# althonos/pyskani

Measured on AMD Instinct MI355X. Metric: genome-pairs/sec (sketch+ANI), higher is better.
Workload: dtype u64; 1 GPU; all-vs-all 10000 x 10000 synthetic ~5 Mb genomes on one GPU (100 families x 100; single-contig genomes, substitutions only), c=125 marker_c=1000 k=15; device-resident ASCII; hits=999867, genomes=10000, parallelism=references sharded over 1 GPU(s)

## Files before the change

pyskani_amd/csrc/slice_join.hip:

```cpp
#include "slice_join.h"
#include "chain_dev.h"

void gsl_make_tab(const BatchQ* bq, size_t n_entries, const uint32_t* q_seeds, std::vector<uint2>& tab, std::vector<uint2>& ebase, uint64_t* n_records, uint64_t* n_slices) {
    tab.clear(); ebase.resize(n_entries);
    uint64_t rec = 0, nsl_all = 0; uint32_t max_sl = 0;
    for (size_t e = 0; e < n_entries; e++) {
        const uint32_t nsl = (q_seeds[e] + GSL_SEEDS - 1) / GSL_SEEDS;
        ebase[e] = make_uint2((uint32_t)rec, (uint32_t)nsl_all);
        rec += (uint64_t)nsl * (bq[e].rank_hi - bq[e].rank_lo);
        nsl_all += nsl;
        max_sl = std::max(max_sl, nsl);
    }
    *n_records = rec; *n_slices = nsl_all;
    (void)max_sl;
    for (size_t e = 0; e < n_entries; e++) for (uint32_t sl = 0; sl < (q_seeds[e] + GSL_SEEDS - 1) / GSL_SEEDS; sl++) tab.push_back(make_uint2((uint32_t)e, sl));
}

#ifndef GSL_LINE_N
#define GSL_LINE_N 4
#endif
constexpr uint32_t GSL_LW = GSL_LINE_N, GSL_LM = GSL_LW - 1u, GSL_LS = GSL_LW == 8 ? 3u : GSL_LW == 4 ? 2u : 1u;
static_assert(GSL_LW == 8 || GSL_LW == 4 || GSL_LW == 2, "a staged line holds eight, four or two anchors");
static size_t gsl_walk_lds(const GslArgs& A, bool emit) {
    const size_t nw = (A.n_refs + 63) / 64;
    (void)nw;
    return (emit ? (8 * GSL_LW + 8 + 8) * (size_t)A.p_cap + 8 * 64 : 0) + 64 + 4 * (size_t)A.p_cap + (emit ? 0 : 4 * (size_t)GSL_WORDS * (A.p_cap + 1));
}

__device__ __forceinline__ uint32_t gsl_ref_word(unsigned long long v) { return (uint32_t)(v >> 53) & 7u; }
__device__ __forceinline__ uint32_t gsl_ref_bit(unsigned long long v) { return (uint32_t)(v >> 48) & 31u; }
__device__ __forceinline__ uint32_t gsl_tag(unsigned long long v) { return (uint32_t)(v >> 56); }
template <bool EMIT, bool TAGGED>
__global__ __launch_bounds__(64) void gsl_walk_kernel(GslArgs A) {
    extern __shared__ uint4 s_gsl[];
    const int lane = threadIdx.x;
    const uint2 te = A.tab[blockIdx.x];
    if (te.x == 0xFFFFFFFFu) return;
    if (EMIT && (A.err[5] || *(const unsigned long long*)(A.err + 16) > A.cap)) return;
    const BatchQ B = A.bq[te.x];
    const SketchDesc Q = A.qd[B.q];
    const uint32_t sb = te.y * GSL_SEEDS;
    if (sb >= Q.n) return;
    const uint32_t se = Q.n - sb > GSL_SEEDS ? sb + GSL_SEEDS : Q.n;
    const uint32_t P = B.rank_hi - B.rank_lo, pc = A.p_cap;
    const uint2 eb = A.ebase[te.x];
    const uint32_t rec0 = eb.x + te.y * P;
    uint2* s_line = (uint2*)s_gsl;
    unsigned long long* s_lim = (unsigned long long*)(s_line + (EMIT ? GSL_LW * pc : 0u));
    uint2* s_cs = (uint2*)(s_lim + (EMIT ? pc : 0u));
    uint2* s_fl = s_cs + (EMIT ? pc : 0u);
    uint2* s_bp = s_fl + (EMIT ? 64u : 0u);
    uint32_t* s_cur = (uint32_t*)(s_bp + 8u);
    uint32_t* s_rows = s_cur;
    uint32_t* s_bm = s_cur + pc;
    {
        if (EMIT) for (uint32_t j = lane; j < P; j += 64) { const uint4 v = A.rec[rec0 + j]; s_cs[j] = make_uint2(v.x, v.x); s_rows[j] = v.y; s_lim[j] = ((unsigned long long)v.w << 32) | v.z; }
        else {
            for (uint32_t j = lane; j < P; j += 64) s_cur[j] = 0;
            for (uint32_t x = lane; x < GSL_WORDS * (pc + 1u); x += 64) s_bm[x] = 0;
        }
    }
    uint32_t unw = 0;
    if (EMIT && lane < (int)GSL_WORDS) unw = A.un[(size_t)(eb.y + te.y) * GSL_WORDS + lane];
    lds_wave_sync();
    constexpr uint32_t GSL_AHEAD = 4;
    unsigned long long visited = 0;
    const uint32_t n_blk = A.blk_cnt[te.x];
    const uint32_t* __restrict__ brow = A.blk_tab + (size_t)te.x * A.blk_cap * GSL_BT_WORDS;
#pragma unroll 1
    for (uint32_t bi = 0; bi < n_blk; bi++, brow += GSL_BT_WORDS) {
    {
    const uint32_t blk = brow[8];
    const unsigned long long x_base = ((unsigned long long)brow[11] << 32) | brow[10];
    const uint32_t* __restrict__ x_key = A.g_key + x_base; const unsigned long long* __restrict__ x_val = A.g_val + x_base;
    {
        lds_wave_sync();
        if (lane < 8) {
            uint32_t run = brow[9];
#pragma unroll
            for (int u = 0; u < 7; u++) { const uint32_t w = brow[u]; if (u < lane) run += (uint32_t)__popc(w); }
            s_bp[lane] = make_uint2(brow[lane], run);
        }
        lds_wave_sync();
    }
    const uint32_t* __restrict__ bkt = A.g_bucket + (size_t)blk * A.g_nb1;
    uint32_t km1 = sb + (uint32_t)lane < se ? Q.kmer[sb + lane] : 0u, km2 = sb + 64u + (uint32_t)lane < se ? Q.kmer[sb + 64u + lane] : 0u;
    uint32_t lo1 = 0, hi1 = 0;
    if (sb + (uint32_t)lane < se) { const uint32_t b = km1 >> A.g_shift; lo1 = bkt[b]; hi1 = bkt[b + 1]; }
    for (uint32_t c0 = sb; c0 < se; c0 += 64) {
        const uint32_t i = c0 + (uint32_t)lane;
        const uint32_t km = km1, lo = lo1, hi = hi1;
        km1 = km2; lo1 = 0; hi1 = 0;
        if (i + 64u < se) { const uint32_t b = km1 >> A.g_shift; lo1 = bkt[b]; hi1 = bkt[b + 1]; }
        km2 = i + 128u < se ? Q.kmer[i + 128u] : 0u;
        uint32_t qp = 0, qm = 0;
        if (EMIT && i < se) { qp = Q.pos[i]; qm = Q.meta[i]; }
        const uint32_t nst = (hi - lo + 63u) >> 6;
        if (!EMIT) visited += hi - lo;
        uint32_t pre = nst;
#pragma unroll
        for (int o = 1; o < 64; o <<= 1) { const uint32_t y = __shfl_up(pre, o); if (lane >= o) pre += y; }
        const uint32_t T = (uint32_t)__builtin_amdgcn_readlane((int)pre, 63);
        pre -= nst;
        uint32_t ns[GSL_AHEAD], nx[GSL_AHEAD], nh[GSL_AHEAD], nk[GSL_AHEAD]; unsigned long long nv[GSL_AHEAD];
#define GSL_FETCH(t, u) do { \
            ns[u] = 0; nx[u] = 0; nh[u] = 0; nk[u] = 0xFFFFFFFFu; nv[u] = 0ull; \
            if ((t) < T) { \
                const unsigned long long own = __ballot(nst != 0 && pre <= (t)); \
                ns[u] = 63u - (uint32_t)__clzll((long long)own); \
                nx[u] = (uint32_t)__builtin_amdgcn_readlane((int)lo, (int)ns[u]) + 64u * ((t) - (uint32_t)__builtin_amdgcn_readlane((int)pre, (int)ns[u])); \
                nh[u] = (uint32_t)__builtin_amdgcn_readlane((int)hi, (int)ns[u]); \
                if (nx[u] + (uint32_t)lane < nh[u]) { if (!TAGGED) nk[u] = x_key[nx[u] + lane]; nv[u] = x_val[nx[u] + lane]; } \
            } } while (0)
#pragma unroll
        for (uint32_t u = 0; u < GSL_AHEAD; u++) GSL_FETCH(u, u);
        for (uint32_t t0 = 0; t0 < T; t0 += GSL_AHEAD) {
            uint32_t cs[GSL_AHEAD], cx[GSL_AHEAD], ch[GSL_AHEAD], ck[GSL_AHEAD]; unsigned long long cv[GSL_AHEAD];
#pragma unroll
            for (uint32_t u = 0; u < GSL_AHEAD; u++) { cs[u] = ns[u]; cx[u] = nx[u]; ch[u] = nh[u]; ck[u] = nk[u]; cv[u] = nv[u]; }
#pragma unroll
            for (uint32_t u = 0; u < GSL_AHEAD; u++) GSL_FETCH(t0 + GSL_AHEAD + u, u);
            uint32_t slots[GSL_AHEAD]; uint2 bps[GSL_AHEAD];
#pragma unroll
            for (uint32_t u = 0; u < GSL_AHEAD; u++) bps[u] = s_bp[gsl_ref_word(cv[u])];
#pragma unroll
            for (uint32_t u = 0; u < GSL_AHEAD; u++) {
                const uint32_t skm = (uint32_t)__builtin_amdgcn_readlane((int)km, (int)cs[u]);
                const uint32_t b = gsl_ref_bit(cv[u]), rk = bps[u].y + (uint32_t)__popc(bps[u].x & ~(~0u << b)) - B.rank_lo;
                const bool hit = TAGGED ? gsl_tag(cv[u]) == (skm & 0xFFu) : ck[u] == skm;
                const bool ok = cx[u] + (uint32_t)lane < ch[u] && hit && ((bps[u].x >> b) & 1u) && rk < P;
                slots[u] = ok ? rk : 0xFFFFFFFFu;
            }
#pragma unroll
            for (uint32_t u = 0; u < GSL_AHEAD; u++) {
                if (t0 + u >= T) break;
                const uint32_t s = cs[u]; const unsigned long long v = cv[u];
                const uint32_t slot = slots[u];
                const bool valid = slot != 0xFFFFFFFFu;
                if (!__any(valid)) continue;
                const uint32_t jl = c0 - sb + s;
                if (!EMIT) {
                    if (valid) { atomicAdd(&s_cur[slot], 1u); atomicOr(&s_bm[(jl >> 5) * (pc + 1u) + slot], 1u << (jl & 31u)); }
                    continue;
                }
                const uint32_t sqp = (uint32_t)__builtin_amdgcn_readlane((int)qp, (int)s), sqm = (uint32_t)__builtin_amdgcn_readlane((int)qm, (int)s);
                const uint32_t rmeta = (uint32_t)((((v >> 33) & ((1ull << GSI_CONTIG_BITS) - 1ull)) << 1) | (v & 1ull));
                const uint32_t prev = (uint32_t)__builtin_amdgcn_update_dpp(-1, (int)slot, 0x138 , 0xf, 0xf, false);
                const bool same = valid && prev == slot;
                const bool dup = __ballot(same) != 0;
                const uint2 cs = s_cs[valid ? slot : 0u];
                const unsigned long long lim = s_lim[valid ? slot : 0u];
                const uint32_t base = cs.x;
                bool opens = false;
                if (((uint32_t)__builtin_amdgcn_readlane((int)unw, (int)(jl >> 5)) >> (jl & 31u)) & 1u) {
                    const unsigned long long key1 = (((unsigned long long)(sqm >> 1) << 32) | sqp) + 1ull;
                    opens = valid && key1 > lim;
                    if (opens && !same) {
                        const uint32_t row = s_rows[slot], idxc = base < A.cap ? base : A.cap;
                        if (row < Q.rows) {
                            const size_t ri = (size_t)B.row_off + (size_t)slot * Q.rows + row;
                            uint2* r = A.chunks + ri;
                            r->x = idxc;
                            if (row > 0) r[-1].y = idxc;
                            A.row_q0[ri] = make_uint2(sqp, sqm >> 1);
                        } else atomicOr(A.err, 1u);
                        s_rows[slot] = row + 1u; s_lim[slot] = key1 + FRAGMENT_LENGTH;
                    }
                }
                const uint32_t q_rel = opens ? 0u : sqp - (uint32_t)(lim - 1ull - FRAGMENT_LENGTH);
                const uint2 av = pk_anchor(q_rel, (uint32_t)(v >> 1), (rmeta & ~1u) | ((rmeta ^ sqm) & 1u));
                if (!dup) {
                    const uint32_t t3 = base & GSL_LM;
                    if (valid) { s_cs[slot].x = base + 1u; s_line[t3 * pc + slot] = av; }
                    const bool fl = valid && t3 == GSL_LM;
                    const unsigned long long fm = __ballot(fl);
                    if (fm) {
                        if (fl) {
                            const uint32_t st0 = cs.y, lb = base & ~GSL_LM, ft = lb >= st0 ? 0u : st0 - lb;
                            s_fl[__popcll(fm & ((1ull << lane) - 1ull))] = make_uint2(slot | (ft << 16), lb);
                        }
                        lds_wave_sync();
                        const uint32_t nf = (uint32_t)__popcll(fm), t = (uint32_t)lane & GSL_LM;
                        for (uint32_t g0 = 0; g0 < nf; g0 += 64u / GSL_LW) {
                            const uint32_t r2 = g0 + ((uint32_t)lane >> GSL_LS);
                            if (r2 < nf) { const uint2 f = s_fl[r2]; if (t >= (f.x >> 16)) A.anc[f.y + t] = s_line[t * pc + (f.x & 0xFFFFu)]; }
                        }
                    }
                    continue;
                }
                const uint32_t st0 = cs.y;
                const uint32_t next = (uint32_t)__builtin_amdgcn_update_dpp(-1, (int)slot, 0x130 , 0xf, 0xf, false);
                const bool last = valid && next != slot;
                const unsigned long long starts = __ballot(valid && !same);
                const unsigned long long upto = starts & (lane == 63 ? ~0ull : ((2ull << lane) - 1ull));
                const uint32_t jj = valid ? (uint32_t)lane - (63u - (uint32_t)__clzll((long long)upto)) : 0u;
                const unsigned long long ends = __ballot(last);
                const uint32_t tail = valid ? (uint32_t)__ffsll((long long)(ends >> lane)) - 1u : 0u;
                const uint32_t d = base + jj, e = d + tail, lastline = e >> GSL_LS;
                if (valid && jj == 0 && (base >> GSL_LS) != lastline && e < A.cap) {
                    const uint32_t f0 = (base & ~GSL_LM) > st0 ? (base & ~GSL_LM) : st0;
                    for (uint32_t t = f0; t < base; t++) A.anc[t] = s_line[(t & GSL_LM) * pc + slot];
                }
                lds_wave_sync();
                if (valid) {
                    if ((d >> GSL_LS) == lastline) s_line[(d & GSL_LM) * pc + slot] = av;
                    else if (e < A.cap) A.anc[d] = av;
                }
                lds_wave_sync();
                if (last) {
                    if (e >= A.cap) atomicOr(A.err, 2u);
                    else if ((e & GSL_LM) == GSL_LM) {
                        const uint32_t f0 = (e & ~GSL_LM) > st0 ? (e & ~GSL_LM) : st0;
                        for (uint32_t t = f0; t <= e; t++) A.anc[t] = s_line[(t & GSL_LM) * pc + slot];
                    }
                    s_cs[slot].x = e + 1u;
                }
                lds_wave_sync();
            }
        }
#undef GSL_FETCH
    }
    }
    }
    lds_wave_sync();
    if (!EMIT) {
#pragma unroll
        for (int o = 32; o > 0; o >>= 1) visited += __shfl_xor(visited, o);
        if (lane == 0 && visited) atomicAdd((unsigned long long*)(A.err + 18), visited);
        for (uint32_t j = lane; j < P; j += 64) {
            const uint32_t c = s_cur[j];
            A.cnt[rec0 + j] = c;
            if (c) atomicAdd(&A.pair_cnt[B.pair_off + j], c);
        }
        for (uint32_t x = lane; x < P * GSL_WORDS; x += 64) { const uint32_t j = x / GSL_WORDS, w = x % GSL_WORDS; A.bm[(size_t)(rec0 + j) * GSL_WORDS + w] = s_bm[w * (pc + 1u) + j]; }
    } else {
        for (uint32_t j = lane; j < P; j += 64) {
            const uint32_t c = s_cs[j].x, st0 = s_cs[j].y;
            if (c > st0 && (c & GSL_LM) && c <= A.cap) {
                const uint32_t f0 = ((c - 1u) & ~GSL_LM) > st0 ? ((c - 1u) & ~GSL_LM) : st0;
                for (uint32_t t = f0; t < c; t++) A.anc[t] = s_line[(t & GSL_LM) * pc + j];
            }
        }
    }
}

constexpr uint32_t GSL_HK = GSL_SEEDS / 64;
__global__ __launch_bounds__(64) void gsl_heads_kernel(GslArgs A) {
    __shared__ unsigned long long s_key[GSL_SEEDS];
    __shared__ uint32_t s_bm[64 * (GSL_WORDS + 1)];
    __shared__ uint32_t s_un[GSL_WORDS];
    const int lane = threadIdx.x;
    const uint32_t e = blockIdx.x;
    const BatchQ B = A.bq[e];
    const uint32_t P = B.rank_hi - B.rank_lo, j = blockIdx.y * 64u + (uint32_t)lane;
    if (blockIdx.y * 64u >= P) return;
    const SketchDesc Q = A.qd[B.q];
    const bool act = j < P;
    const uint32_t nsl = (Q.n + GSL_SEEDS - 1u) / GSL_SEEDS;
    const uint32_t p = B.pair_off + j;
    const uint2 eb = A.ebase[e];
    const bool guard = A.err[5] || *(const unsigned long long*)(A.err + 16) > A.cap;
    uint32_t cursor = act ? A.pstart[p] : 0u;
    const uint32_t pend = act ? A.pstart[p + 1] : 0u;
    const bool live = act && !guard && pend - cursor >= MIN_ANCHORS;
    uint32_t rows = 0; unsigned long long lim1 = live ? 0ull : ~0ull;
    uint32_t* my_bm = s_bm + lane * (GSL_WORDS + 1);
    struct HSlice { uint32_t kp[GSL_HK], kmt[GSL_HK]; uint4 bw[GSL_WORDS / 4]; uint32_t c; };
    HSlice S0, S1;
    auto load_slice = [&](HSlice& X, uint32_t sl) {
        const uint32_t sb = sl * GSL_SEEDS;
#pragma unroll
        for (uint32_t u = 0; u < GSL_HK; u++) { const uint32_t i = sb + u * 64u + (uint32_t)lane; X.kp[u] = 0; X.kmt[u] = 0; if (i < Q.n) { X.kp[u] = Q.pos[i]; X.kmt[u] = Q.meta[i]; } }
        const size_t r = (size_t)eb.x + (size_t)sl * P + j;
        X.c = 0;
#pragma unroll
        for (uint32_t u = 0; u < GSL_WORDS / 4; u++) X.bw[u] = make_uint4(0, 0, 0, 0);
        if (act) {
            X.c = A.cnt[r];
            const uint4* __restrict__ src = (const uint4*)(A.bm + r * GSL_WORDS);
#pragma unroll
            for (uint32_t u = 0; u < GSL_WORDS / 4; u++) X.bw[u] = src[u];
        }
    };
    auto step = [&](HSlice& X, uint32_t sl) {
        const uint32_t sb = sl * GSL_SEEDS, ns = Q.n - sb > GSL_SEEDS ? GSL_SEEDS : Q.n - sb;
        const size_t r = (size_t)eb.x + (size_t)sl * P + j;
        lds_wave_sync();
        if (lane < (int)GSL_WORDS) s_un[lane] = 0;
#pragma unroll
        for (uint32_t u = 0; u < GSL_HK; u++) s_key[u * 64u + lane] = (((unsigned long long)(X.kmt[u] >> 1) << 32) | X.kp[u]) + 1ull;
#pragma unroll
        for (uint32_t u = 0; u < GSL_WORDS / 4; u++) { my_bm[4 * u] = X.bw[u].x; my_bm[4 * u + 1] = X.bw[u].y; my_bm[4 * u + 2] = X.bw[u].z; my_bm[4 * u + 3] = X.bw[u].w; }
        const uint32_t c = X.c;
        if (sl + 2 < nsl) load_slice(X, sl + 2);
        lds_wave_sync();
        if (act) {
            A.rec[r] = make_uint4(cursor, rows, (uint32_t)lim1, (uint32_t)(lim1 >> 32));
            if (live && c) {
                uint32_t from = 0;
                for (;;) {
                    {
                        uint32_t lo = from, hi = ns;
                        while (lo < hi) { const uint32_t mid = (lo + hi) >> 1; if (s_key[mid] > lim1) hi = mid; else lo = mid + 1; }
                        from = lo;
                    }
                    if (from >= ns) break;
                    uint32_t w = from >> 5, x = my_bm[w] & (~0u << (from & 31u));
                    while (!x && ++w < GSL_WORDS) x = my_bm[w];
                    if (!x) break;
                    const uint32_t jl = w * 32u + (uint32_t)__ffs((int)x) - 1u;
                    lim1 = s_key[jl] + FRAGMENT_LENGTH; rows++;
                    atomicOr(&s_un[w], 1u << (jl & 31u));
                    from = jl + 1u;
                }
            }
            cursor += c;
        }
        lds_wave_sync();
        if (lane < (int)GSL_WORDS && s_un[lane]) atomicOr(&A.un[(size_t)(eb.y + sl) * GSL_WORDS + lane], s_un[lane]);
    };
    load_slice(S0, 0);
    if (nsl > 1) load_slice(S1, 1);
    for (uint32_t sl = 0; sl < nsl; sl += 2) {
        step(S0, sl);
        if (sl + 1 < nsl) step(S1, sl + 1);
    }
    if (act) {
        if (live && rows) {
            if (rows - 1u < Q.rows) A.chunks[(size_t)B.row_off + (size_t)j * Q.rows + rows - 1u].y = pend < A.cap ? pend : A.cap; else atomicOr(A.err, 1u);
        }
        A.n_chunks[p] = live ? (rows < Q.rows ? rows : Q.rows) : 0u;
    }
}

__global__ __launch_bounds__(64) void gsl_blocks_kernel(const BatchQ* __restrict__ bq, uint32_t n_entries, const uint8_t* __restrict__ pass, uint32_t n_refs, uint32_t g_blocks,
                                                        const unsigned long long* __restrict__ g_base, uint32_t* __restrict__ blk_tab, uint32_t* __restrict__ blk_cnt, uint32_t blk_cap) {
    static_assert(BSI_BLOG == 8, "four ballots of 64 references = one index block");
    const uint32_t e = blockIdx.x;
    if (e >= n_entries) return;
    const int lane = threadIdx.x;
    const BatchQ B = bq[e];
    const uint8_t* __restrict__ row = pass + (size_t)B.q * n_refs;
    uint32_t* __restrict__ out = blk_tab + (size_t)e * blk_cap * GSL_BT_WORDS;
    uint32_t run = 0, cnt = 0;
    for (uint32_t blk = 0; blk < g_blocks && run < B.rank_hi; blk++) {
        uint8_t f[4];
#pragma unroll
        for (int u = 0; u < 4; u++) { const uint32_t r = (blk * 4u + u) * 64u + (uint32_t)lane; f[u] = r < n_refs ? row[r] : (uint8_t)0; }
        unsigned long long m[4]; uint32_t n_here = 0;
#pragma unroll
        for (int u = 0; u < 4; u++) { m[u] = __ballot(f[u] != 0); n_here += (uint32_t)__popcll(m[u]); }
        if (n_here && run + n_here > B.rank_lo) {
            if (cnt < blk_cap) {
                uint32_t w = 0;
#pragma unroll
                for (int u = 0; u < 4; u++) { if (lane == 2 * u) w = (uint32_t)m[u]; if (lane == 2 * u + 1) w = (uint32_t)(m[u] >> 32); }
                const unsigned long long base = g_base[blk];
                if (lane == 8) w = blk; if (lane == 9) w = run; if (lane == 10) w = (uint32_t)base; if (lane == 11) w = (uint32_t)(base >> 32);
                if (lane < (int)GSL_BT_WORDS) out[(size_t)cnt * GSL_BT_WORDS + lane] = w;
            }
            cnt++;
        }
        run += n_here;
    }
    if (lane == 0) blk_cnt[e] = cnt < blk_cap ? cnt : blk_cap;
}
psk_status gsl_blocks_launch(const BatchQ* bq, uint32_t n_entries, const uint8_t* pass, uint32_t n_refs, uint32_t g_blocks, const unsigned long long* g_base,
                             uint32_t* blk_tab, uint32_t* blk_cnt, uint32_t blk_cap, hipStream_t st) {
    if (!n_entries) return PSK_OK;
    hipLaunchKernelGGL(gsl_blocks_kernel, dim3(n_entries), dim3(64), 0, st, bq, n_entries, pass, n_refs, g_blocks, g_base, blk_tab, blk_cnt, blk_cap);
    PSK_HIP(hipGetLastError());
    return PSK_OK;
}
psk_status gsl_count_launch(const GslArgs& A, hipStream_t st) {
    auto* const walk = A.tagged ? gsl_walk_kernel<false, true> : gsl_walk_kernel<false, false>;
    hipLaunchKernelGGL(walk, dim3(A.n_tab), dim3(64), gsl_walk_lds(A, false), st, A);
    PSK_HIP(hipGetLastError());
    return PSK_OK;
}
psk_status gsl_heads_launch(const GslArgs& A, hipStream_t st) {
    PSK_HIP(hipMemsetAsync(A.un, 0, 4 * (size_t)GSL_WORDS * A.n_slices, st));
    hipLaunchKernelGGL(gsl_heads_kernel, dim3(A.n_entries, (A.p_cap + 63u) / 64u), dim3(64), 0, st, A);
    PSK_HIP(hipGetLastError());
    return PSK_OK;
}
psk_status gsl_emit_launch(const GslArgs& A, hipStream_t st) {
    auto* const walk = A.tagged ? gsl_walk_kernel<true, true> : gsl_walk_kernel<true, false>;
    hipLaunchKernelGGL(walk, dim3(A.n_tab), dim3(64), gsl_walk_lds(A, true), st, A);
    PSK_HIP(hipGetLastError());
    return PSK_OK;
}
```

Measured before the change: 220.2 million genome-pairs/s.

## Precompute per-block slot lookup table and iterate buckets with ballot mask

Replaces the per-hit rank computation (bitmask word plus popcount prefix) with a 256-entry LDS table of 16-bit slots built once per block using mbcnt, so each candidate does a single LDS lookup. The bucket walk drops the wave-wide prefix scan and per-step ballot search and instead walks a pending-lane mask with ctz. In the count pass it caches the query k-mer at bucket switch and clamps loads in place of predicating them. These changes target per-candidate ALU and cross-lane overhead, at the cost of more LDS and possibly less even chunk scheduling.

```diff
diff --git a/pyskani_amd/csrc/slice_join.hip b/pyskani_amd/csrc/slice_join.hip
--- a/pyskani_amd/csrc/slice_join.hip
+++ b/pyskani_amd/csrc/slice_join.hip
@@ -24,11 +24,10 @@
 static size_t gsl_walk_lds(const GslArgs& A, bool emit) {
     const size_t nw = (A.n_refs + 63) / 64;
     (void)nw;
-    return (emit ? (8 * GSL_LW + 8 + 8) * (size_t)A.p_cap + 8 * 64 : 0) + 64 + 4 * (size_t)A.p_cap + (emit ? 0 : 4 * (size_t)GSL_WORDS * (A.p_cap + 1));
-}
-
-__device__ __forceinline__ uint32_t gsl_ref_word(unsigned long long v) { return (uint32_t)(v >> 53) & 7u; }
-__device__ __forceinline__ uint32_t gsl_ref_bit(unsigned long long v) { return (uint32_t)(v >> 48) & 31u; }
+    return (emit ? (8 * GSL_LW + 8 + 8) * (size_t)A.p_cap + 8 * 64 : 0) + 512 + 4 * (size_t)A.p_cap + (emit ? 0 : 4 * (size_t)GSL_WORDS * (A.p_cap + 1));
+}
+
+__device__ __forceinline__ uint32_t gsl_ref(unsigned long long v) { return (uint32_t)(v >> 48) & 0xFFu; }
 __device__ __forceinline__ uint32_t gsl_tag(unsigned long long v) { return (uint32_t)(v >> 56); }
 template <bool EMIT, bool TAGGED>
 __global__ __launch_bounds__(64) void gsl_walk_kernel(GslArgs A) {
@@ -49,8 +48,8 @@
     unsigned long long* s_lim = (unsigned long long*)(s_line + (EMIT ? GSL_LW * pc : 0u));
     uint2* s_cs = (uint2*)(s_lim + (EMIT ? pc : 0u));
     uint2* s_fl = s_cs + (EMIT ? pc : 0u);
-    uint2* s_bp = s_fl + (EMIT ? 64u : 0u);
-    uint32_t* s_cur = (uint32_t*)(s_bp + 8u);
+    uint16_t* s_slot = (uint16_t*)(s_fl + (EMIT ? 64u : 0u));
+    uint32_t* s_cur = (uint32_t*)(s_slot + 256u);
     uint32_t* s_rows = s_cur;
     uint32_t* s_bm = s_cur + pc;
     {
@@ -75,11 +74,14 @@
     const uint32_t* __restrict__ x_key = A.g_key + x_base; const unsigned long long* __restrict__ x_val = A.g_val + x_base;
     {
         lds_wave_sync();
-        if (lane < 8) {
-            uint32_t run = brow[9];
-#pragma unroll
-            for (int u = 0; u < 7; u++) { const uint32_t w = brow[u]; if (u < lane) run += (uint32_t)__popc(w); }
-            s_bp[lane] = make_uint2(brow[lane], run);
+        uint32_t run = brow[9] - B.rank_lo;
+#pragma unroll
+        for (uint32_t u = 0; u < 4; u++) {
+            const uint32_t w0 = brow[2 * u], w1 = brow[2 * u + 1];
+            const uint32_t rk = run + __builtin_amdgcn_mbcnt_hi(w1, __builtin_amdgcn_mbcnt_lo(w0, 0u));
+            const bool pass = (((unsigned long long)w1 << 32 | w0) >> lane) & 1ull;
+            s_slot[64u * u + (uint32_t)lane] = pass && rk < P ? (uint16_t)rk : (uint16_t)0xFFFFu;
+            run += (uint32_t)__popc(w0) + (uint32_t)__popc(w1);
         }
         lds_wave_sync();
     }
@@ -97,43 +99,44 @@
         if (EMIT && i < se) { qp = Q.pos[i]; qm = Q.meta[i]; }
         const uint32_t nst = (hi - lo + 63u) >> 6;
         if (!EMIT) visited += hi - lo;
-        uint32_t pre = nst;
-#pragma unroll
-        for (int o = 1; o < 64; o <<= 1) { const uint32_t y = __shfl_up(pre, o); if (lane >= o) pre += y; }
-        const uint32_t T = (uint32_t)__builtin_amdgcn_readlane((int)pre, 63);
-        pre -= nst;
-        uint32_t ns[GSL_AHEAD], nx[GSL_AHEAD], nh[GSL_AHEAD], nk[GSL_AHEAD]; unsigned long long nv[GSL_AHEAD];
-#define GSL_FETCH(t, u) do { \
-            ns[u] = 0; nx[u] = 0; nh[u] = 0; nk[u] = 0xFFFFFFFFu; nv[u] = 0ull; \
-            if ((t) < T) { \
-                const unsigned long long own = __ballot(nst != 0 && pre <= (t)); \
-                ns[u] = 63u - (uint32_t)__clzll((long long)own); \
-                nx[u] = (uint32_t)__builtin_amdgcn_readlane((int)lo, (int)ns[u]) + 64u * ((t) - (uint32_t)__builtin_amdgcn_readlane((int)pre, (int)ns[u])); \
-                nh[u] = (uint32_t)__builtin_amdgcn_readlane((int)hi, (int)ns[u]); \
-                if (nx[u] + (uint32_t)lane < nh[u]) { if (!TAGGED) nk[u] = x_key[nx[u] + lane]; nv[u] = x_val[nx[u] + lane]; } \
-            } } while (0)
-#pragma unroll
-        for (uint32_t u = 0; u < GSL_AHEAD; u++) GSL_FETCH(u, u);
-        for (uint32_t t0 = 0; t0 < T; t0 += GSL_AHEAD) {
-            uint32_t cs[GSL_AHEAD], cx[GSL_AHEAD], ch[GSL_AHEAD], ck[GSL_AHEAD]; unsigned long long cv[GSL_AHEAD];
-#pragma unroll
-            for (uint32_t u = 0; u < GSL_AHEAD; u++) { cs[u] = ns[u]; cx[u] = nx[u]; ch[u] = nh[u]; ck[u] = nk[u]; cv[u] = nv[u]; }
-#pragma unroll
-            for (uint32_t u = 0; u < GSL_AHEAD; u++) GSL_FETCH(t0 + GSL_AHEAD + u, u);
-            uint32_t slots[GSL_AHEAD]; uint2 bps[GSL_AHEAD];
-#pragma unroll
-            for (uint32_t u = 0; u < GSL_AHEAD; u++) bps[u] = s_bp[gsl_ref_word(cv[u])];
+        constexpr bool KM_AT_SWITCH = !EMIT;
+        unsigned long long pending = __ballot(nst != 0);
+        uint32_t it_s = 0, it_x = 0, it_h = 0, it_k = 0;
+        uint32_t ns[GSL_AHEAD], nx[GSL_AHEAD], nh[GSL_AHEAD], nk[GSL_AHEAD], nkm[GSL_AHEAD]; unsigned long long nv[GSL_AHEAD];
+#define GSL_FETCH(u) do { \
+            if (it_x >= it_h) { \
+                if (pending) { \
+                    it_s = (uint32_t)__builtin_ctzll(pending); pending &= pending - 1ull; \
+                    it_x = (uint32_t)__builtin_amdgcn_readlane((int)lo, (int)it_s); it_h = (uint32_t)__builtin_amdgcn_readlane((int)hi, (int)it_s); \
+                    if (KM_AT_SWITCH) it_k = (uint32_t)__builtin_amdgcn_readlane((int)km, (int)it_s); \
+                } else { it_s = 0; it_x = 0; it_h = 0; } \
+            } \
+            ns[u] = it_s; nx[u] = it_x; nh[u] = it_h; nkm[u] = it_k; nk[u] = 0xFFFFFFFFu; nv[u] = 0ull; \
+            if (EMIT) { if (nx[u] + (uint32_t)lane < nh[u]) { if (!TAGGED) nk[u] = x_key[nx[u] + lane]; nv[u] = x_val[nx[u] + lane]; } } \
+            else { const uint32_t ix = nx[u] + (uint32_t)lane < nh[u] ? nx[u] + (uint32_t)lane : nx[u]; if (!TAGGED) nk[u] = x_key[ix]; nv[u] = x_val[ix]; } \
+            it_x += 64u; \
+            } while (0)
+#pragma unroll
+        for (uint32_t u = 0; u < GSL_AHEAD; u++) GSL_FETCH(u);
+        for (;;) {
+            uint32_t cs[GSL_AHEAD], cx[GSL_AHEAD], ch[GSL_AHEAD], ck[GSL_AHEAD], ckm[GSL_AHEAD]; unsigned long long cv[GSL_AHEAD];
+#pragma unroll
+            for (uint32_t u = 0; u < GSL_AHEAD; u++) { cs[u] = ns[u]; cx[u] = nx[u]; ch[u] = nh[u]; ck[u] = nk[u]; cv[u] = nv[u]; ckm[u] = nkm[u]; }
+            if (ch[0] == 0) break;
+#pragma unroll
+            for (uint32_t u = 0; u < GSL_AHEAD; u++) GSL_FETCH(u);
+            uint32_t slots[GSL_AHEAD], sl[GSL_AHEAD];
+#pragma unroll
+            for (uint32_t u = 0; u < GSL_AHEAD; u++) sl[u] = s_slot[gsl_ref(cv[u])];
 #pragma unroll
             for (uint32_t u = 0; u < GSL_AHEAD; u++) {
-                const uint32_t skm = (uint32_t)__builtin_amdgcn_readlane((int)km, (int)cs[u]);
-                const uint32_t b = gsl_ref_bit(cv[u]), rk = bps[u].y + (uint32_t)__popc(bps[u].x & ~(~0u << b)) - B.rank_lo;
+                const uint32_t skm = KM_AT_SWITCH ? ckm[u] : (uint32_t)__builtin_amdgcn_readlane((int)km, (int)cs[u]);
                 const bool hit = TAGGED ? gsl_tag(cv[u]) == (skm & 0xFFu) : ck[u] == skm;
-                const bool ok = cx[u] + (uint32_t)lane < ch[u] && hit && ((bps[u].x >> b) & 1u) && rk < P;
-                slots[u] = ok ? rk : 0xFFFFFFFFu;
+                slots[u] = cx[u] + (uint32_t)lane < ch[u] && hit && sl[u] != 0xFFFFu ? sl[u] : 0xFFFFFFFFu;
             }
 #pragma unroll
             for (uint32_t u = 0; u < GSL_AHEAD; u++) {
-                if (t0 + u >= T) break;
+                if (ch[u] == 0) break;
                 const uint32_t s = cs[u]; const unsigned long long v = cv[u];
                 const uint32_t slot = slots[u];
                 const bool valid = slot != 0xFFFFFFFFu;
```

Result: faster. 226.7 million genome-pairs/s (median of 6 runs) (+2.9%).
